# world-modelz/world-modelz

Measured on AMD Instinct MI355X. Metric: denoise-step latent-frames/sec (forward, 32x16x16 latent clips), higher is better.
Workload: dtype bf16; 1 GPU; BASELINE.json configs[3] per GPU: VqVideoDiffusionModel.forward, B=8 clips/GPU of 32x16x16 latents, codebook 1024, dim 256, dim_head 128, heads 1, extents 3,3,3, depth 4, mlp 256; clips_per_gpu=8, codebook=1024, parallelism=clips sharded over 1 rank(s), no data-path collective

## Files before the change

### world_modelz_amd/csrc/attn_fwd_row16_infer.hip

```cpp
#include "attn_common.h"

#ifdef WMZ_OP16_F16
#error "attn_fwd_row16_infer.hip is a bfloat16 unit"
#endif

namespace {

constexpr int DH = 128, NW = 16, KCR = 8, RS = 2;
constexpr int KROW = DH * 2 + 32, VROW = DH * 2 + 32;
constexpr int KIMG = KCR * 16 * KROW, VIMG = KCR * 16 * VROW, BUF = KIMG + VIMG;
constexpr int PK = KIMG / 1024, PV = VIMG / 1024;
static_assert(PK == 36 && PV == 36, "pieces 0 and 1 exist for every wave, piece 2 for waves 0 .. 3");
constexpr int KS = DH / 32, MT = DH / 16;
constexpr float DEFER = 8.f;
constexpr unsigned LD_B = 128u * 2u;
constexpr unsigned ROW_B = 16u * LD_B;
constexpr long PLANE_B = 256l * LD_B;

__device__ __forceinline__ unsigned div_m31(unsigned n, unsigned m) { return __umulhi(n << 1, m); }
unsigned magic_m31(unsigned d) { return (unsigned)(((1ull << 31) + d - 1) / d); }

template <int EH, int EW>
__global__ __launch_bounds__(NW * 64, 4) void attn_fwd_row16_infer_kernel(const bf16_t* __restrict__ Q, const bf16_t* __restrict__ K,
                                                                        const bf16_t* __restrict__ V, bf16_t* __restrict__ O,
                                                                        int S, int eS, int qs0, int Sq, float scale,
                                                                        unsigned m_sq, unsigned m_win) {
  static_assert(EH == 3 || EH == 1, "the steps of a slab are written out for these row extents");
  __shared__ __attribute__((aligned(1024))) char smem[2 * BUF];
  const int tid = threadIdx.x, lane = tid & 63;
  const int wave = __builtin_amdgcn_readfirstlane(tid >> 6);
  const int g = lane >> 4, li = lane & 15;

  const unsigned xcd = blockIdx.x & 7u;
  const unsigned lid = xcd * (gridDim.x >> 3) + min(xcd, gridDim.x & 7u) + (blockIdx.x >> 3);
  const int b = (int)div_m31(lid, m_sq);
  const int sq = (int)(lid - (unsigned)b * (unsigned)Sq);
  const int s = qs0 + sq;
  const int hq = wave;
  const unsigned tok_q = (unsigned)(b * S + s) * 256u + (unsigned)(hq * 16);
  const unsigned tok_o = lid * 256u + (unsigned)(hq * 16);
  const float c2 = scale * 1.4426950408889634f;

  float bm[4];
#pragma unroll
  for (int r = 0; r < 4; ++r) {
    const int d = 4 * g + r - li;
    bm[r] = (d <= EW && -d <= EW) ? 0.f : -INFINITY;
  }

  Frag8<bf16_t> qf[KS];
  f32x4 o[MT];
#pragma unroll
  for (int mt = 0; mt < MT; ++mt) o[mt] = (f32x4)(0.f);
  float m_run = 0.f, l_run = 0.f;
  float thr = -INFINITY;

  const int kbase = li * KROW + g * 16;
  const int vbase = KIMG + (4 * g + (li >> 2)) * VROW + (li & 3) * 8;
  const int my_lo = max(hq - EH, 0), my_hi = min(hq + EH, 15);
  const int lo0 = max(0, (my_lo + RS - 1) >> 1), hi0 = min(KCR - 1, my_hi >> 1);
  const int lo1 = max(0, (my_lo - 1 + RS - 1) >> 1), hi1 = min(KCR - 1, (my_hi - 1) >> 1);
  const bool has2 = wave + 2 * NW < PK;

  unsigned kvo[3], vvo[3];
#pragma unroll
  for (int i = 0; i < 3; ++i) kvo[i] = piece_voff<DH, KROW, RS>(wave + NW * i, lane, LD_B, 16 - RS);
#pragma unroll
  for (int i = 0; i < 3; ++i) vvo[i] = piece_voff<DH, VROW, RS>(wave + NW * i, lane, LD_B, 16 - RS);

  const int sk_lo = max(0, s - eS), sk_hi = min(S - 1, s + eS);
  const int nplanes = sk_hi - sk_lo + 1;
  const int nwin = 2 * eS + 1;
  int p_first = s - eS;
  {
    const unsigned d = (unsigned)(S - 1 - p_first);
    p_first += (int)(d - div_m31(d, m_win) * (unsigned)nwin);
  }
  if (p_first > sk_hi || p_first < sk_lo) p_first = sk_lo;
  const unsigned long pl_b = (unsigned long)(unsigned)(b * S + p_first) * (unsigned long)PLANE_B;
  const char* kpl = (const char*)K + pl_b;
  const char* vpl = (const char*)V + pl_b;
  const int t_wrap = sk_hi - p_first;
  const long back = -(long)(nplanes - 1) * PLANE_B;

  int wdst = wave * 1024;
  auto issue_k = [&](auto par, auto ic, const char* kp) {
    constexpr int PAR = decltype(par)::value, i = decltype(ic)::value;
    __builtin_amdgcn_global_load_lds((gptr_t)((kp + PAR * ROW_B) + kvo[i]), (lptr_t)(smem + wdst + PAR * BUF + i * NW * 1024), 16, 0, 0);
  };
  auto issue_v = [&](auto par, auto ic, const char* vp) {
    constexpr int PAR = decltype(par)::value, i = decltype(ic)::value;
    __builtin_amdgcn_global_load_lds((gptr_t)((vp + PAR * ROW_B) + vvo[i]), (lptr_t)(smem + wdst + PAR * BUF + KIMG + i * NW * 1024), 16, 0, 0);
  };
  using C0 = std::integral_constant<int, 0>;
  using C1 = std::integral_constant<int, 1>;
  using C2 = std::integral_constant<int, 2>;

  auto rescale = [&](float mx, auto& t) {
    constexpr int nt = (int)(sizeof(t) / sizeof(float));
    float gm = wave_groups_max(mx);
    gm = fmaxf(gm, thr - DEFER);
    const float alpha = __builtin_amdgcn_exp2f(fminf(-gm, 0.f));
    l_run *= alpha;
#pragma unroll
    for (int mt = 0; mt < MT; ++mt) o[mt] *= alpha;
    thr = DEFER;
    m_run += gm;
#pragma unroll
    for (int r = 0; r < 4; ++r) bm[r] = (bm[r] == -INFINITY) ? -INFINITY : -m_run;
#pragma unroll
    for (int r = 0; r < nt; ++r) t[r] -= gm;
  };

  auto step2 = [&](auto par, int t0, bool vnow, const char* vp) {
    constexpr int PAR = decltype(par)::value;
    using NX = std::integral_constant<int, 1 - PAR>;
    const char* Sb = smem + PAR * BUF;
    const int ko = kbase + t0 * 16 * KROW;
    const unsigned va0 = lds_addr(Sb + vbase + t0 * 16 * VROW), va1 = va0 + 16 * VROW;
    f32x4 sc0 = (f32x4)(0.f), sc1 = (f32x4)(0.f);
#pragma unroll
    for (int ks = 0; ks < KS; ++ks) {
      Frag8<bf16_t> ka, kb;
      ka.v = *reinterpret_cast<const s16x8*>(Sb + ko + ks * 64);
      kb.v = *reinterpret_cast<const s16x8*>(Sb + ko + 16 * KROW + ks * 64);
      mma16(sc0, ka, qf[ks]);
      mma16(sc1, kb, qf[ks]);
    }
    __builtin_amdgcn_sched_barrier(0);
    s16x4 x0[MT], x1[MT];
    static_for<MT>([&](auto mt) {
      x0[mt] = ds_read_tr16_asm<mt * 32>(va0);
      x1[mt] = ds_read_tr16_asm<mt * 32>(va1);
    });
    if (vnow) issue_v(NX{}, C0{}, vp);
    float t[8];
#pragma unroll
    for (int r = 0; r < 4; ++r) {
      t[r] = fmaf(sc0[r], c2, bm[r]);
      t[4 + r] = fmaf(sc1[r], c2, bm[r]);
    }
    const float mx = fmaxf(__builtin_fmaxf(__builtin_fmaxf(t[0], t[1]), __builtin_fmaxf(t[2], t[3])),
                           __builtin_fmaxf(__builtin_fmaxf(t[4], t[5]), __builtin_fmaxf(t[6], t[7])));
    if (__any(mx > thr)) rescale(mx, t);
    float p[8];
    Frag8<bf16_t> pf;
#pragma unroll
    for (int r = 0; r < 8; ++r) p[r] = __builtin_amdgcn_exp2f(t[r]);
    l_run += ((p[0] + p[1]) + (p[2] + p[3])) + ((p[4] + p[5]) + (p[6] + p[7]));
    frag_from_f32<bf16_t>(pf, p);
    if (vnow) issue_v(NX{}, C1{}, vp);
    ds_tr_wait();
#pragma unroll
    for (int mt = 0; mt < MT; ++mt) {
      asm volatile("" : "+v"(x0[mt]), "+v"(x1[mt]));
      Frag8<bf16_t> vf;
      vf.v = __builtin_shufflevector(x0[mt], x1[mt], 0, 1, 2, 3, 4, 5, 6, 7);
      mma16(o[mt], vf, pf);
    }
  };
  auto step1 = [&](auto par, int t0) {
    constexpr int PAR = decltype(par)::value;
    const char* Sb = smem + PAR * BUF;
    const int ko = kbase + t0 * 16 * KROW;
    const unsigned va0 = lds_addr(Sb + vbase + t0 * 16 * VROW);
    f32x4 sc0 = (f32x4)(0.f);
#pragma unroll
    for (int ks = 0; ks < KS; ++ks) {
      Frag8<bf16_t> ka;
      ka.v = *reinterpret_cast<const s16x8*>(Sb + ko + ks * 64);
      mma16(sc0, ka, qf[ks]);
    }
    __builtin_amdgcn_sched_barrier(0);
    s16x4 x0[MT];
    static_for<MT>([&](auto mt) { x0[mt] = ds_read_tr16_asm<mt * 32>(va0); });
    float t[4];
#pragma unroll
    for (int r = 0; r < 4; ++r) t[r] = fmaf(sc0[r], c2, bm[r]);
    const float mx = __builtin_fmaxf(__builtin_fmaxf(t[0], t[1]), __builtin_fmaxf(t[2], t[3]));
    if (__any(mx > thr)) rescale(mx, t);
    float p[4];
#pragma unroll
    for (int r = 0; r < 4; ++r) p[r] = __builtin_amdgcn_exp2f(t[r]);
    l_run += (p[0] + p[1]) + (p[2] + p[3]);
    s16x4 pf;
#pragma unroll
    for (int r = 0; r < 4; ++r) pf[r] = (short)f32_to_bf16_bits(p[r]);
    ds_tr_wait();
#pragma unroll
    for (int mt = 0; mt < MT; ++mt) {
      asm volatile("" : "+v"(x0[mt]));
      o[mt] = op16_mfma_16x16x16(x0[mt], pf, o[mt]);
    }
  };
  auto slab = [&](auto par, bool more, const char* kp, const char* vp) {
    constexpr int PAR = decltype(par)::value;
    using NX = std::integral_constant<int, 1 - PAR>;
    asm volatile("" : "+s"(wdst), "+v"(kvo[0]), "+v"(kvo[1]), "+v"(kvo[2]), "+v"(vvo[0]), "+v"(vvo[1]), "+v"(vvo[2]));
    asm volatile("s_waitcnt vmcnt(0)" ::: "memory");
    __builtin_amdgcn_s_barrier();
    if (more) {
      issue_k(NX{}, C0{}, kp); issue_k(NX{}, C1{}, kp);
      if (has2) issue_k(NX{}, C2{}, kp);
    }
    const int lo = PAR ? lo1 : lo0, hi = PAR ? hi1 : hi0;
    if constexpr (EH == 3) {
      int t0 = lo;
      bool vnow = more;
#pragma clang loop unroll(disable)
      do { step2(par, t0, vnow, vp); vnow = false; t0 += 2; } while (t0 + 1 <= hi);
      if (t0 <= hi) step1(par, t0);
    } else {
      int t0 = lo;
      if (t0 < hi) { step2(par, t0, more, vp); t0 += 2; }
      if (t0 <= hi) {
        step1(par, t0);
        if (more) { issue_v(NX{}, C0{}, vp); issue_v(NX{}, C1{}, vp); }
      }
    }
    if (more && has2) issue_v(NX{}, C2{}, vp);
  };

  issue_k(C0{}, C0{}, kpl); issue_k(C0{}, C1{}, kpl);
  issue_v(C0{}, C0{}, vpl); issue_v(C0{}, C1{}, vpl);
  if (has2) { issue_k(C0{}, C2{}, kpl); issue_v(C0{}, C2{}, vpl); }
  {
    const bf16_t* qrow = Q + (unsigned long)tok_q * 128ul + (unsigned)(li * 128);
#pragma unroll
    for (int ks = 0; ks < KS; ++ks) frag_load(qf[ks], qrow + ks * 32 + g * 8);
  }
#pragma unroll
  for (int ks = 0; ks < KS; ++ks) asm volatile("" : "+v"(qf[ks].v));
  int t = 0;
  do {
    slab(C0{}, true, kpl, vpl);
    const long mv = t == t_wrap ? back : PLANE_B;
    kpl += mv; vpl += mv;
    slab(C1{}, t + 1 < nplanes, kpl, vpl);
  } while (++t < nplanes);

  {
    float l = wave_groups_sum(l_run);
    const float inv = 1.f / l;
    bf16_t* orow = O + (unsigned long)tok_o * 128ul + (unsigned)(li * 128);
#pragma unroll
    for (int mt = 0; mt < MT; mt += 2) {
      unsigned a0 = (unsigned)f32_to_bf16_bits(o[mt][0] * inv) | ((unsigned)f32_to_bf16_bits(o[mt][1] * inv) << 16);
      unsigned a1 = (unsigned)f32_to_bf16_bits(o[mt][2] * inv) | ((unsigned)f32_to_bf16_bits(o[mt][3] * inv) << 16);
      unsigned b0 = (unsigned)f32_to_bf16_bits(o[mt + 1][0] * inv) | ((unsigned)f32_to_bf16_bits(o[mt + 1][1] * inv) << 16);
      unsigned b1 = (unsigned)f32_to_bf16_bits(o[mt + 1][2] * inv) | ((unsigned)f32_to_bf16_bits(o[mt + 1][3] * inv) << 16);
      const auto s0 = __builtin_amdgcn_permlane16_swap(a0, b0, false, false);
      const auto s1 = __builtin_amdgcn_permlane16_swap(a1, b1, false, false);
      i32x4 pk;
      pk[0] = (int)s0[0]; pk[1] = (int)s1[0]; pk[2] = (int)s0[1]; pk[3] = (int)s1[1];
      const int col = (g & 1) ? (mt + 1) * 16 + 4 * (g - 1) : mt * 16 + 4 * g;
      *reinterpret_cast<i32x4*>(orow + col) = pk;
    }
  }
}

template <int EH, int EW>
int launch_infer(const void* q, const void* k, const void* v, void* out, const AttnGeom& G, hipStream_t st) {
  const long nwg = (long)G.B * G.Sq;
  hipLaunchKernelGGL((attn_fwd_row16_infer_kernel<EH, EW>), dim3((unsigned)nwg), dim3(NW * 64), 0, st, (const bf16_t*)q,
                     (const bf16_t*)k, (const bf16_t*)v, (bf16_t*)out, G.S, G.eS, G.qs0, G.Sq, G.scale,
                     magic_m31((unsigned)G.Sq), magic_m31(2u * (unsigned)G.eS + 1u));
  WMZ_LAUNCH_CHECK("wmz_local3d_attn_fwd(row16 infer)");
  return WMZ_OK;
}

}

bool wmz_attn_fwd_row16_infer_takes(const AttnGeom& G) {
  return G.W == 16 && G.H == 16 && G.dh == 128 && G.heads == 1 && G.ldq == 128 && G.ldk == 128 && G.ldv == 128 && G.ldo == 128 &&
         ((G.eH == 3 && G.eW == 3) || (G.eH == 1 && G.eW == 1)) && G.dbg == 0 && G.variant == 0 && G.w8 == 0 &&
         (long)G.B * G.S * 256 <= (1l << 31) && (long)G.B * G.Sq * G.Sq <= (1l << 31) && ((long)G.S + G.eS) * (2l * G.eS + 1) <= (1l << 31);
}

int wmz_attn_fwd_row16_infer_dispatch(const void* q, const void* k, const void* v, void* out, const AttnGeom& G, hipStream_t st) {
  if (G.eH == 3) return launch_infer<3, 3>(q, k, v, out, G, st);
  return launch_infer<1, 1>(q, k, v, out, G, st);
}
```

### world_modelz_amd/csrc/attn_slab_walk.h

```cpp
#pragma once
#ifdef __HIPCC__
#define WMZ_HD __host__ __device__ __forceinline__
#else
#define WMZ_HD inline
#endif

WMZ_HD int slab_min(int a, int b) { return a < b ? a : b; }
WMZ_HD int slab_max(int a, int b) { return a > b ? a : b; }
constexpr int slab_log2(int n) { return n <= 1 ? 0 : 1 + slab_log2(n >> 1); }

struct SlabGeom { int H, s_last, t_lo, t_hi, sk_lo, sk_hi, c_first, nch, nslab; };

WMZ_HD int slab_first_plane(const SlabGeom& g, int eS, int s) {
  const int nwin = 2 * eS + 1;
  int p_first = s - eS;
  { const int a = (((g.s_last - p_first) % nwin) + nwin) % nwin; p_first += a; }
  if (p_first > g.sk_hi || p_first < g.sk_lo) p_first = g.sk_lo;
  return p_first;
}

template <int CH, int KC, bool CLAMP = true>
WMZ_HD SlabGeom slab_geom(int H, int S, int eS, int eHv, int h0, int NW, int s) {
  constexpr int RS = CH / KC, LOG_CH = slab_log2(CH);
  static_assert(KC * RS == CH && (1 << LOG_CH) == CH && (1 << slab_log2(RS)) == RS, "a slab is one phase of a chunk of 2^n rows");
  SlabGeom g;
  g.H = H;
  g.t_lo = slab_max(h0 - eHv, 0);
  g.t_hi = slab_min((CLAMP ? slab_min(h0 + NW - 1, H - 1) : h0 + NW - 1) + eHv, H - 1);
  g.sk_lo = slab_max(0, s - eS); g.s_last = S - 1; g.sk_hi = slab_min(g.s_last, s + eS);
  g.c_first = g.t_lo >> LOG_CH;
  g.nch = ((g.t_hi >> LOG_CH) - g.c_first + 1) * RS;
  g.nslab = (g.sk_hi - g.sk_lo + 1) * g.nch;
  return g;
}

template <int CH, int KC, bool CLAMP = true> struct SlabWalk {
  static constexpr int RS = CH / KC, LOG_RS = slab_log2(RS), LOG_CH = slab_log2(CH);
  int pl, rem = 0, base = 0, j = 0, bsafe = 0, dlim = CH - RS;
  WMZ_HD SlabWalk(const SlabGeom& g, int p_first) : pl(p_first - g.sk_lo) {}
  WMZ_HD void next_state(const SlabGeom& g) {
    base = ((g.c_first + (rem >> LOG_RS)) << LOG_CH) + (rem & (RS - 1));
    bsafe = CLAMP ? slab_min(base, g.H - 1) : base;
    if (CLAMP) dlim = slab_max(g.H - 1 - base, 0);
  }
  template <typename Move> WMZ_HD void advance(const SlabGeom& g, Move move_planes) {
    ++j;
    if (++rem == g.nch) {
      rem = 0;
      if (g.sk_lo + pl == g.sk_hi) { move_planes(-(long)pl); pl = 0; }
      else { ++pl; move_planes(1); }
    }
  }
};

WMZ_HD int w32_row_lo(int R, int eH) { return R - (R & 1) - 2 * eH; }
WMZ_HD int w32_row_hi(int R, int eH) { return R - (R & 1) + 2 * eH + 1; }
WMZ_HD int w32_dw(int R, int c, int Rk, int ck) { return 16 * ((Rk & 1) - (R & 1)) + ck - c; }
WMZ_HD int w32_dh(int R, int Rk) { return (Rk - R + (R & 1) - (Rk & 1)) / 2; }
WMZ_HD bool w32_col_ok(int R, int c, int Rk, int ck, int eW) { const int d = w32_dw(R, c, Rk, ck); return d <= eW && -d <= eW; }
WMZ_HD int w32_stage_extent(int eH) { return 2 * eH; }

template <int DH, int ROWP, int RS>
WMZ_HD unsigned piece_voff(int piece, int lane, unsigned ld_bytes, int row_lim) {
  const int off = piece * 1024 + lane * 16;
  const int r = off / ROWP;
  int c = (off - r * ROWP) >> 4;
  c = c < DH / 8 ? c : 0;
  const int prow = slab_min(RS * (r >> 4), row_lim);
  return (unsigned)((prow << 4) + (r & 15)) * ld_bytes + (unsigned)c * 16u;
}
```

### world_modelz_amd/csrc/wmz_debug.h

```cpp
#pragma once
#ifdef __cplusplus
extern "C" {
#endif

int wmz_debug_fused_timestamps(void* buf);
int wmz_debug_fused_knobs(int dbg);
int wmz_debug_attn_timestamps(void* buf);
int wmz_debug_attn_knobs(int dbg, int variant);

int wmz_debug_conv_knobs(int skew, int dbg);

int wmz_debug_linear_knobs(int dma);
int wmz_debug_linear_route(const void* A, long lda, const void* Wt, long block_stride, int M, int N, int K, int prologue,
                           int out_f32, int dtype);

int wmz_debug_stamp(void* buf, int slot, void* stream);

int wmz_debug_conv_stamps(unsigned long long* out, int n);
int wmz_debug_w3_stamps(unsigned long long* out, int n);

#ifdef __cplusplus
}
#endif
```

Baseline: 795,500 latent-frames/s.

## Remap wave rows and rebalance K/V async loads onto lightly loaded waves

For the 3-row-extent attention inference kernel, waves are remapped to query rows (swapping neighbouring rows in alternate groups of four). The next slab's K and V images are now issued only by waves whose rows have fewer than four key rows of the current parity, each loading four 1 KB pieces of K and V at fixed class offsets, instead of every wave issuing its own pieces interleaved with compute. The goal is to move the load-issue work off the busiest waves so the slowest wave per slab finishes sooner. Optional timestamp instrumentation is also added behind a compile flag. The new piece-to-class mapping must cover the same image exactly, and mistakes there would corrupt the loaded K/V data.

```diff
diff --git a/world_modelz_amd/csrc/attn_fwd_row16_infer.hip b/world_modelz_amd/csrc/attn_fwd_row16_infer.hip
--- a/world_modelz_amd/csrc/attn_fwd_row16_infer.hip
+++ b/world_modelz_amd/csrc/attn_fwd_row16_infer.hip
@@ -2,6 +2,24 @@
 
 #ifdef WMZ_OP16_F16
 #error "attn_fwd_row16_infer.hip is a bfloat16 unit"
+#endif
+#ifndef WMZ_ATTN_ROWMAP
+#define WMZ_ATTN_ROWMAP 1
+#endif
+#ifndef WMZ_ATTN_PLAN
+#define WMZ_ATTN_PLAN 1
+#endif
+#ifdef WMZ_ATTN_INFER_TS
+__device__ unsigned long long attn_infer_stamps[16 * 64];
+#define WMZ_ITS(slot) do { if (blockIdx.x == 0 && lane == 0) attn_infer_stamps[wave * 64 + (slot)] = __builtin_readcyclecounter(); } while (0)
+#define WMZ_ITS_REAL(slot) do { if (blockIdx.x == 0 && lane == 0) attn_infer_stamps[wave * 64 + (slot)] = __builtin_amdgcn_s_memrealtime(); } while (0)
+#define WMZ_ITS_SLAB(k) do { if (its_j < 14) WMZ_ITS((k) + 4 * its_j); } while (0)
+#define WMZ_ITS_NEXT() (void)++its_j
+#else
+#define WMZ_ITS(slot) do { } while (0)
+#define WMZ_ITS_REAL(slot) do { } while (0)
+#define WMZ_ITS_SLAB(k) do { } while (0)
+#define WMZ_ITS_NEXT() do { } while (0)
 #endif
 
 namespace {
@@ -20,6 +38,20 @@
 __device__ __forceinline__ unsigned div_m31(unsigned n, unsigned m) { return __umulhi(n << 1, m); }
 unsigned magic_m31(unsigned d) { return (unsigned)(((1ull << 31) + d - 1) / d); }
 
+constexpr unsigned long issue_classes(bool rowmap) {
+  unsigned long t = 0;
+  for (int w = 0; w < NW; ++w) {
+    const int c = slab_issue_class(rowmap ? slab_wave_row(w) : w);
+    t |= (unsigned long)(c < 0 ? 0 : c) << (4 * w);
+  }
+  return t;
+}
+constexpr unsigned issuers(bool rowmap, int par) {
+  unsigned m = 0;
+  for (int w = 0; w < NW; ++w) m |= (unsigned)slab_issues(rowmap ? slab_wave_row(w) : w, par) << w;
+  return m;
+}
+
 template <int EH, int EW>
 __global__ __launch_bounds__(NW * 64, 4) void attn_fwd_row16_infer_kernel(const bf16_t* __restrict__ Q, const bf16_t* __restrict__ K,
                                                                         const bf16_t* __restrict__ V, bf16_t* __restrict__ O,
@@ -30,13 +62,19 @@
   const int tid = threadIdx.x, lane = tid & 63;
   const int wave = __builtin_amdgcn_readfirstlane(tid >> 6);
   const int g = lane >> 4, li = lane & 15;
+#ifdef WMZ_ATTN_INFER_TS
+  int its_j = 0;
+#endif
+  WMZ_ITS(0); WMZ_ITS_REAL(60);
 
   const unsigned xcd = blockIdx.x & 7u;
   const unsigned lid = xcd * (gridDim.x >> 3) + min(xcd, gridDim.x & 7u) + (blockIdx.x >> 3);
   const int b = (int)div_m31(lid, m_sq);
   const int sq = (int)(lid - (unsigned)b * (unsigned)Sq);
   const int s = qs0 + sq;
-  const int hq = wave;
+  constexpr bool ROWMAP = EH == 3 && WMZ_ATTN_ROWMAP, PLAN = EH == 3 && WMZ_ATTN_PLAN;
+  int hq = wave;
+  if constexpr (ROWMAP) hq = slab_wave_row(wave);
   const unsigned tok_q = (unsigned)(b * S + s) * 256u + (unsigned)(hq * 16);
   const unsigned tok_o = lid * 256u + (unsigned)(hq * 16);
   const float c2 = scale * 1.4426950408889634f;
@@ -84,6 +122,22 @@
   const long back = -(long)(nplanes - 1) * PLANE_B;
 
   int wdst = wave * 1024;
+  static_assert(KROW == VROW, "one offset register serves both images");
+  int cdst = 0;
+  unsigned pvo = 0;
+  bool iss0 = false, iss1 = false;
+  if constexpr (PLAN) {
+    constexpr unsigned long CLS = issue_classes(ROWMAP);
+    constexpr unsigned ISS0 = issuers(ROWMAP, 0), ISS1 = issuers(ROWMAP, 1);
+    const int cls = (int)(CLS >> (4 * wave)) & 15;
+    iss0 = (ISS0 >> wave) & 1u; iss1 = (ISS1 >> wave) & 1u;
+    pvo = piece_voff<DH, KROW, RS>(cls, lane, LD_B, 16 - RS);
+    cdst = cls * 1024;
+  }
+  auto issue_c = [&](auto par, auto jc, int img, const char* p) {
+    constexpr int PAR = decltype(par)::value, j = decltype(jc)::value;
+    __builtin_amdgcn_global_load_lds((gptr_t)((p + PAR * ROW_B) + (pvo + j * SLAB_CLASS_STEP)), (lptr_t)(smem + cdst + PAR * BUF + img + j * 9 * 1024), 16, 0, 0);
+  };
   auto issue_k = [&](auto par, auto ic, const char* kp) {
     constexpr int PAR = decltype(par)::value, i = decltype(ic)::value;
     __builtin_amdgcn_global_load_lds((gptr_t)((kp + PAR * ROW_B) + kvo[i]), (lptr_t)(smem + wdst + PAR * BUF + i * NW * 1024), 16, 0, 0);
@@ -196,17 +250,26 @@
   auto slab = [&](auto par, bool more, const char* kp, const char* vp) {
     constexpr int PAR = decltype(par)::value;
     using NX = std::integral_constant<int, 1 - PAR>;
-    asm volatile("" : "+s"(wdst), "+v"(kvo[0]), "+v"(kvo[1]), "+v"(kvo[2]), "+v"(vvo[0]), "+v"(vvo[1]), "+v"(vvo[2]));
+    if constexpr (PLAN) asm volatile("" : "+s"(cdst), "+v"(pvo));
+    else asm volatile("" : "+s"(wdst), "+v"(kvo[0]), "+v"(kvo[1]), "+v"(kvo[2]), "+v"(vvo[0]), "+v"(vvo[1]), "+v"(vvo[2]));
     asm volatile("s_waitcnt vmcnt(0)" ::: "memory");
+    WMZ_ITS_SLAB(3);
     __builtin_amdgcn_s_barrier();
-    if (more) {
+    WMZ_ITS_SLAB(4);
+    if constexpr (PLAN) {
+      if (more && (PAR ? iss1 : iss0)) {
+        static_for<4>([&](auto j) { issue_c(NX{}, j, 0, kp); });
+        static_for<4>([&](auto j) { issue_c(NX{}, j, KIMG, vp); });
+      }
+    } else if (more) {
       issue_k(NX{}, C0{}, kp); issue_k(NX{}, C1{}, kp);
       if (has2) issue_k(NX{}, C2{}, kp);
     }
+    WMZ_ITS_SLAB(5);
     const int lo = PAR ? lo1 : lo0, hi = PAR ? hi1 : hi0;
     if constexpr (EH == 3) {
       int t0 = lo;
-      bool vnow = more;
+      bool vnow = more && !PLAN;
 #pragma clang loop unroll(disable)
       do { step2(par, t0, vnow, vp); vnow = false; t0 += 2; } while (t0 + 1 <= hi);
       if (t0 <= hi) step1(par, t0);
@@ -218,12 +281,14 @@
         if (more) { issue_v(NX{}, C0{}, vp); issue_v(NX{}, C1{}, vp); }
       }
     }
-    if (more && has2) issue_v(NX{}, C2{}, vp);
+    if (!PLAN && more && has2) issue_v(NX{}, C2{}, vp);
+    WMZ_ITS_SLAB(6); WMZ_ITS_NEXT();
   };
 
   issue_k(C0{}, C0{}, kpl); issue_k(C0{}, C1{}, kpl);
   issue_v(C0{}, C0{}, vpl); issue_v(C0{}, C1{}, vpl);
   if (has2) { issue_k(C0{}, C2{}, kpl); issue_v(C0{}, C2{}, vpl); }
+  WMZ_ITS(2);
   {
     const bf16_t* qrow = Q + (unsigned long)tok_q * 128ul + (unsigned)(li * 128);
 #pragma unroll
@@ -238,6 +303,7 @@
     kpl += mv; vpl += mv;
     slab(C1{}, t + 1 < nplanes, kpl, vpl);
   } while (++t < nplanes);
+  WMZ_ITS(63);
 
   {
     float l = wave_groups_sum(l_run);
@@ -257,6 +323,7 @@
       *reinterpret_cast<i32x4*>(orow + col) = pk;
     }
   }
+  WMZ_ITS(62); WMZ_ITS_REAL(61);
 }
 
 template <int EH, int EW>
@@ -277,6 +344,12 @@
          (long)G.B * G.S * 256 <= (1l << 31) && (long)G.B * G.Sq * G.Sq <= (1l << 31) && ((long)G.S + G.eS) * (2l * G.eS + 1) <= (1l << 31);
 }
 
+#ifdef WMZ_ATTN_INFER_TS
+extern "C" int wmz_debug_attn_infer_stamps(unsigned long long* out, int n) {
+  return (int)hipMemcpyFromSymbol(out, HIP_SYMBOL(attn_infer_stamps), (size_t)n * sizeof(unsigned long long));
+}
+#endif
+
 int wmz_attn_fwd_row16_infer_dispatch(const void* q, const void* k, const void* v, void* out, const AttnGeom& G, hipStream_t st) {
   if (G.eH == 3) return launch_infer<3, 3>(q, k, v, out, G, st);
   return launch_infer<1, 1>(q, k, v, out, G, st);
diff --git a/world_modelz_amd/csrc/attn_slab_walk.h b/world_modelz_amd/csrc/attn_slab_walk.h
--- a/world_modelz_amd/csrc/attn_slab_walk.h
+++ b/world_modelz_amd/csrc/attn_slab_walk.h
@@ -60,6 +60,17 @@
 WMZ_HD bool w32_col_ok(int R, int c, int Rk, int ck, int eW) { const int d = w32_dw(R, c, Rk, ck); return d <= eW && -d <= eW; }
 WMZ_HD int w32_stage_extent(int eH) { return 2 * eH; }
 
+constexpr int slab_wave_row(int wave) { return wave ^ ((wave >> 2) & 1); }
+constexpr int slab_rows_of_parity(int row, int eH, int par, int H = 16) {
+  const int lo = row - eH > 0 ? row - eH : 0, hi = row + eH < H - 1 ? row + eH : H - 1;
+  return (hi - par + 2) / 2 - (lo - par + 1) / 2;
+}
+constexpr unsigned SLAB_CLASS_STEP = 16384u;
+constexpr int slab_issue_class(int row) {
+  return row <= 2 ? row : row >= 13 ? row - 10 : (row == 4 || row == 11) ? 6 : (row == 6 || row == 9) ? 7 : (row == 7 || row == 8) ? 8 : -1;
+}
+constexpr bool slab_issues(int row, int par) { return slab_issue_class(row) >= 0 && slab_rows_of_parity(row, 3, par) < 4; }
+
 template <int DH, int ROWP, int RS>
 WMZ_HD unsigned piece_voff(int piece, int lane, unsigned ld_bytes, int row_lim) {
   const int off = piece * 1024 + lane * 16;
diff --git a/world_modelz_amd/csrc/wmz_debug.h b/world_modelz_amd/csrc/wmz_debug.h
--- a/world_modelz_amd/csrc/wmz_debug.h
+++ b/world_modelz_amd/csrc/wmz_debug.h
@@ -18,6 +18,7 @@
 
 int wmz_debug_conv_stamps(unsigned long long* out, int n);
 int wmz_debug_w3_stamps(unsigned long long* out, int n);
+int wmz_debug_attn_infer_stamps(unsigned long long* out, int n);
 
 #ifdef __cplusplus
 }
```

After: 806,200 latent-frames/s, median of 6. 1.01x the previous value.
